# Janspiry/Image-Super-Resolution-via-Iterative-Refinement

Hardware: NVIDIA H100
Metric: diffusion steps/sec (batch16, 16->128 SR3) (higher is better)
Workload: dtype bf16

## Files before the change

image-super-resolution-via-iterative-refinement_b200/_native.py:

```python
import ctypes
import os
from ctypes import POINTER, c_char_p, c_double, c_float, c_int, c_int64, c_uint64, c_void_p

import torch

_PKG = os.path.dirname(os.path.abspath(__file__))
LIB_PATH = os.path.join(_PKG, "lib", "libsr3_b200.so")
SR3_MAX_LEVELS = 8
_lib = None


class NativeLibraryError(RuntimeError):
    pass


class UNetConfigC(ctypes.Structure):
    _fields_ = [("in_channel", c_int), ("out_channel", c_int), ("inner_channel", c_int), ("norm_groups", c_int),
                ("n_mults", c_int), ("channel_mults", c_int * SR3_MAX_LEVELS), ("n_attn_res", c_int),
                ("attn_res", c_int * SR3_MAX_LEVELS), ("res_blocks", c_int), ("image_size", c_int), ("channels", c_int),
                ("conditional", c_int), ("precision", c_int)]


PRECISIONS = {"bf16": 0, "fp32": 1}

# ... 66 lines not shown
    "sr3_windowed_begin": (c_int, [c_void_p, c_void_p, c_void_p, c_uint64, c_uint64, c_void_p]),
    "sr3_windowed_set_snapshots": (c_int, [c_void_p, c_void_p, c_int]),
    "sr3_windowed_steps": (c_int, [c_void_p, c_int, c_int, c_void_p, c_void_p]),
    "sr3_windowed_read_state": (c_int, [c_void_p, c_void_p, c_void_p]),
    "sr3_windowed_grid": (c_int, [c_void_p, POINTER(c_int), POINTER(c_int), POINTER(c_int), POINTER(c_int), POINTER(c_float), POINTER(c_float)]),
    "sr3_windowed_profile_step": (c_int, [c_void_p, c_int, c_int, POINTER(c_float), c_void_p]),
    "sr3_windowed_create_range": (c_int, [c_void_p, c_int, c_int, c_int, c_int, c_int, c_int, c_int, c_void_p, POINTER(c_int), POINTER(c_void_p)]),
    "sr3_windowed_phase_begin": (c_int, [c_void_p, c_int, c_void_p]),
    "sr3_windowed_phase_means": (c_int, [c_void_p, c_void_p]),
    "sr3_windowed_phase_merge": (c_int, [c_void_p, c_void_p]),
    "sr3_wstream_create": (c_int, [c_void_p, c_uint64, c_int, c_int, POINTER(c_void_p)]),
    "sr3_wstream_destroy": (None, [c_void_p]),
    "sr3_wstream_admit": (c_int, [c_void_p, POINTER(c_int), c_int, c_void_p, c_void_p, c_int, c_int, c_uint64, POINTER(c_int), c_void_p]),
    "sr3_wstream_step": (c_int, [c_void_p, c_void_p]),
    "sr3_wstream_retire": (c_int, [c_void_p, c_int, c_void_p]),
    "sr3_wstream_slot_state": (c_int, [c_void_p, POINTER(c_int), POINTER(c_int), POINTER(c_int)]),
    "sr3_engine_profile_step": (c_int, [c_void_p, c_int, c_int, c_int, POINTER(c_int), POINTER(c_float), POINTER(c_double), POINTER(c_double),
                                        POINTER(c_int), c_void_p]),
    "sr3_pil_bicubic_tables": (c_int, [c_int, c_int, POINTER(c_int), POINTER(c_int), c_int, POINTER(c_int)]),
    "sr3_resize_bicubic_u8": (c_int, [c_void_p, c_void_p, c_void_p, c_int, c_int, c_int, c_int, c_int, c_int, c_int, c_float, c_float, c_void_p]),
    "sr3_tensor2img": (c_int, [c_void_p, c_void_p, c_int, c_int, c_int, c_int, c_int, c_float, c_float, c_void_p]),
    "sr3_ssd_u8": (c_int, [c_void_p, c_void_p, c_int64, POINTER(c_uint64), c_void_p]),
    "sr3_ssim": (c_int, [c_void_p, c_void_p, c_int, c_int, c_int, c_int, c_int, POINTER(c_double), c_void_p]),
    "sr3_image_metrics": (c_int, [c_void_p, c_void_p, c_int, c_int, c_int, c_int, c_float, c_float, c_void_p, c_void_p, POINTER(c_uint64),
                                  POINTER(c_double), c_void_p]),
    "sr3_engine_num_launches_per_step": (c_int, [c_void_p]),
    "sr3_engine_num_ops_per_step": (c_int, [c_void_p]),
    "sr3_engine_workspace_bytes": (c_int64, [c_void_p]),
    "sr3_engine_read_activation": (c_int, [c_void_p, c_char_p, c_void_p, c_int64, POINTER(c_int64), POINTER(c_int), c_void_p]),
    "sr3_test_read_gradient": (c_int, [c_void_p, c_char_p, c_int, c_void_p, c_int64, POINTER(c_int64), POINTER(c_int), c_void_p]),
    "sr3_bench_conv": (c_int, [c_int, c_int, c_int, c_int, c_int, c_int, c_int, c_int, c_int, c_int, POINTER(c_float)]),
    "sr3_test_gemm": (c_int, [c_void_p, c_void_p, c_void_p, c_int, c_int, c_int, c_int, c_void_p]),
    "sr3_test_attention": (c_int, [c_void_p, c_void_p, c_void_p, c_int, c_int, c_int, c_int, c_void_p]),
    "sr3_test_conv_groupnorm": (c_int, [c_void_p, c_void_p, c_void_p, c_void_p, c_void_p, c_int, c_int, c_void_p, c_void_p, c_int, c_int, c_int, c_int, c_int,
                                        c_int, c_void_p]),
    "sr3_test_conv": (c_int, [c_void_p, c_void_p, c_void_p, c_void_p, c_void_p, c_int, c_int, c_int, c_int, c_int, c_int, c_int,
                              c_void_p]),
    "sr3_test_conv_ex": (c_int, [POINTER(TestConvArgsC), POINTER(GemmGeometryC), c_void_p]),
    "sr3_tile_schedule": (c_int, [c_void_p, c_int, POINTER(GemmGeometryC), POINTER(c_int), POINTER(c_int)]),
    "sr3_test_wgrad": (c_int, [c_void_p, c_void_p, c_void_p, c_int, c_int, c_int, c_int, c_int, c_int, c_int, c_int, c_int, c_int, c_float,
                               c_int, POINTER(c_int), c_void_p]),
    "sr3_test_groupnorm_layer": (c_int, [POINTER(TestGroupNormArgsC), c_void_p]),
    "sr3_test_grad_combine": (c_int, [c_void_p, c_void_p, c_void_p, c_int, c_void_p, c_void_p, c_void_p, c_void_p, c_float, c_int, c_int, c_int,
                                      c_void_p]),
    "sr3_test_dgrad": (c_int, [c_void_p, c_void_p, c_void_p, c_int, c_int, c_int, c_int, c_int, c_int, c_int, c_int, c_void_p]),
    "sr3_test_attention_bwd": (c_int, [c_void_p, c_void_p, c_void_p, c_void_p, c_void_p, c_void_p, c_void_p, c_void_p, c_int, c_int, c_int, c_int,
                                       c_void_p]),
    "sr3_test_film_embed_bwd": (c_int, [POINTER(TestFilmArgsC), c_void_p]),
    "sr3_test_film_embed_fwd": (c_int, [c_void_p] * 10 + [c_int, c_int, c_int, c_void_p]),
    "sr3_test_attention_unfused": (c_int, [c_void_p] * 5 + [c_int] * 5 + [c_void_p]),
    "sr3_test_loss_grad": (c_int, [c_void_p, c_void_p, c_int, c_int, c_int, c_int, c_int, POINTER(c_double), c_void_p, c_int, c_void_p, c_void_p]),
    "sr3_test_grad_load": (c_int, [c_void_p, c_int, c_int, c_int, c_int, c_void_p, c_int, c_void_p, c_void_p]),
    "sr3_test_noise_level_bwd": (c_int, [c_void_p] * 6 + [c_int, c_int, c_void_p]),
    "sr3_test_input_grad": (c_int, [c_void_p, c_void_p, c_void_p, c_int, c_int, c_int, c_int, c_int, c_void_p]),
}
EXPORTED_SYMBOLS = tuple(_SIGS.keys())


def lib():
    global _lib
    if _lib is not None:
        return _lib
    if not os.path.exists(LIB_PATH):
        raise NativeLibraryError(
            f"{LIB_PATH} is missing: run `python -c 'import __graft_entry__ as g; g.build()'` (nvcc, sm_90a). "
            "sr3_b200 has no CPU or eager-PyTorch fallback.")
# ... 603 lines not shown

    def step(self, n=1):
        with torch.cuda.device(self.device):
            for _ in range(int(n)):
                _check(lib().sr3_wstream_step(self._h, _stream()))

    def slot_state(self):
        r, t, st = (c_int * self.slots)(), (c_int * self.slots)(), (c_int * self.slots)()
        _check(lib().sr3_wstream_slot_state(self._h, r, t, st))
        return list(r), list(t), list(st)

    def finished(self):
        r, _, st = self.slot_state()
        return sorted({q for q, v in zip(r, st) if v == 2})

    def retire(self, request):
        with torch.cuda.device(self.device):
            _check(lib().sr3_wstream_retire(self._h, int(request), _stream()))
        return self._canvases.pop(int(request))[0]


def bench_conv(B, H, W, Cin, Cout, k=3, stride=1, resid=False, stats=True, reps=20):
    ms = c_float()
    _check(lib().sr3_bench_conv(B, H, W, Cin, Cout, k, stride, int(resid), int(stats), reps, ctypes.byref(ms)))
    return ms.value


def test_attention(qk_bf16, vT_bf16, nz, Lt, HW, C):
    out = torch.empty(nz * Lt, C, device=qk_bf16.device, dtype=torch.bfloat16)
    _check(lib().sr3_test_attention(_ptr(qk_bf16), _ptr(vT_bf16), _ptr(out), nz, Lt, HW, C, _stream()))
    return out


def test_gemm(a_bf16, b_bf16, block_n):
    M, K = a_bf16.shape
    N = b_bf16.shape[0]
    d = torch.empty(M, N, device=a_bf16.device, dtype=torch.float32)
    _check(lib().sr3_test_gemm(_ptr(a_bf16), _ptr(b_bf16), _ptr(d), M, N, K, block_n, _stream()))
    return d


def test_conv(x_nhwc_bf16, w_oihw, bias, ksize, stride, want_stats=False):
    B, H, W, Cin = x_nhwc_bf16.shape
    Cout = w_oihw.shape[0]
    y = torch.empty(B, H // stride, W // stride, Cout, device=x_nhwc_bf16.device, dtype=torch.float32)
    stats = torch.zeros(B, Cout, 2, device=y.device, dtype=torch.float64) if want_stats else None
    _check(lib().sr3_test_conv(_ptr(x_nhwc_bf16), _ptr(w_oihw), _ptr(bias), _ptr(y), _ptr(stats), B, H, W, Cin, Cout, ksize, stride, _stream()))
    return y, stats


def test_conv_ex(x, w, ksize=3, stride=1, bias=None, bias2=None, resid=None, x2=None, w2=None, want_bf16=False, want_stats=False,
                 fold_up=False, precise=False):
    B, H, W, CX = x.shape
    Cin = CX // 2 if precise else CX
    Cout = w.shape[0]
    OH, OW = (2 * H, 2 * W) if fold_up else (H // stride, W // stride)
    y = torch.empty(B, OH, OW, Cout, device=x.device, dtype=torch.float32)
    yb = torch.empty(B, OH, OW, Cout * (2 if precise else 1), device=x.device, dtype=torch.bfloat16) if want_bf16 else None
    stats = torch.zeros(B, Cout, 2, device=x.device, dtype=torch.float64) if want_stats else None
    keep = [_f32c(t, x.device) if t is not None else None for t in (w, bias, bias2, resid, w2)]
    a = TestConvArgsC()
    a.x, a.w, a.bias, a.bias2, a.resid = x.data_ptr(), *[(t.data_ptr() if t is not None else None) for t in keep[:4]]
    a.x2 = x2.data_ptr() if x2 is not None else None
    a.w2 = keep[4].data_ptr() if keep[4] is not None else None
    a.y, a.y_bf16, a.stats = y.data_ptr(), (yb.data_ptr() if yb is not None else None), (stats.data_ptr() if stats is not None else None)
    a.B, a.H, a.W, a.Cin, a.Cout = B, H, W, Cin, Cout
# ... 183 lines not shown
```

image-super-resolution-via-iterative-refinement_b200/csrc/attn_long_wgmma.cuh:

```cuda
#pragma once
#include "attn_wgmma.cuh"

namespace sr3 {

constexpr int ATTNL_KB = 128;
constexpr int ATTNL_DN = 128;
constexpr int ATTNL_STAGES = 5;
constexpr int ATTNL_STAGE_BYTES = 16384 + 16384;
constexpr int ATTNL_P_BYTES = 128 * ATTNL_KB * 2;
constexpr int ATTNL_SMEM_BYTES = 1024 + GEMM_HDR_BYTES + ATTNL_STAGES * ATTNL_STAGE_BYTES + ATTNL_P_BYTES;

__global__ void __launch_bounds__(ATTN_THREADS, 1) attn_long_kernel(const __grid_constant__ AttnParams p) {
    extern __shared__ uint8_t smem_raw[];
    const uint32_t raw = smem_u32(smem_raw);
    const uint32_t bar_base = (raw + 1023u) & ~1023u;
    const uint32_t base = bar_base + GEMM_HDR_BYTES;
    const uint32_t p_base = base + ATTNL_STAGES * ATTNL_STAGE_BYTES;
    uint8_t* p_ptr = smem_raw + (p_base - raw);
    auto full_bar = [&](int s) { return bar_base + 8u * s; };
    auto empty_bar = [&](int s) { return bar_base + 8u * (ATTNL_STAGES + s); };

    const int n_dc = p.C / ATTNL_DN;
    const int qt = blockIdx.x / n_dc, dc = blockIdx.x % n_dc, z = blockIdx.y;
    const int warp = threadIdx.x >> 5;
    const int lane = threadIdx.x & 31;
    const int kc1 = p.C / 64;
    constexpr int kc3 = ATTNL_KB / 64;
    const int nb = p.Lt / ATTNL_KB;

    if (threadIdx.x == 0) {
        tma_prefetch_desc(&p.qk_map);
        tma_prefetch_desc(&p.vt_map);
        for (int s = 0; s < ATTNL_STAGES; ++s) { mbar_init(full_bar(s), 1); mbar_init(empty_bar(s), 2); }
        fence_mbar_init();
    }
    __syncthreads();
    pdl_launch_dependents();
    pdl_wait();

    if (warp == ATTN_PRODUCER_WARP) {
        int s = 0;
        uint32_t ph = 0;
        auto stage = [&](bool is_s, int kb, int c) {
            mbar_wait(empty_bar(s), ph ^ 1u);
            if (elect_one_sync()) {
// ... 120 lines not shown
```

image-super-resolution-via-iterative-refinement_b200/csrc/attn_wgmma.cuh:

```cuda
#pragma once
#include <cuda_bf16.h>
#include <cuda.h>
#include "gemm_wgmma.cuh"

namespace sr3 {

constexpr int ATTN_THREADS = 288;
constexpr int ATTN_PRODUCER_WARP = 8;
constexpr int ATTN_STAGES = 3;
constexpr int ATTN_STAGE_BYTES = 16384 + 32768;
constexpr int ATTN_P_BYTES = 65536;
constexpr int ATTN_SMEM_BYTES = 1024 + GEMM_HDR_BYTES + ATTN_STAGES * ATTN_STAGE_BYTES + ATTN_P_BYTES;

struct AttnParams {
    CUtensorMap qk_map;
    CUtensorMap vt_map;
    __nv_bfloat16* out;
    int C, Lt, HW, dn, nz;
    float scale_log2e;
};

template <int LT, int DN>
__device__ __forceinline__ void attn_unit_t(const AttnParams& p, const AttnParams* pm, const uint32_t base_in, uint8_t* base_ptr_in,
                                            const int qt, const int dc, const int z) {
    const uint32_t bar_base = base_in;
    const uint32_t base = base_in + GEMM_HDR_BYTES;
    uint8_t* base_ptr = base_ptr_in + GEMM_HDR_BYTES;
    const uint32_t p_base = base + ATTN_STAGES * ATTN_STAGE_BYTES;
    uint8_t* p_ptr = base_ptr + ATTN_STAGES * ATTN_STAGE_BYTES;
    auto full_bar = [&](int s) { return bar_base + 8u * s; };
    auto empty_bar = [&](int s) { return bar_base + 8u * (ATTN_STAGES + s); };

    const int warp = threadIdx.x >> 5;
    const int lane = threadIdx.x & 31;
    const int kc1 = p.C / 64;
    constexpr int kc3 = LT / 64;

    if (threadIdx.x == 0) {
        tma_prefetch_desc(&pm->qk_map);
        tma_prefetch_desc(&pm->vt_map);
        for (int s = 0; s < ATTN_STAGES; ++s) { mbar_init(full_bar(s), 1); mbar_init(empty_bar(s), 2); }
        fence_mbar_init();
    }
    __syncthreads();
    pdl_launch_dependents();
    pdl_wait();

    if (warp == ATTN_PRODUCER_WARP) {
        int s = 0;
        uint32_t ph = 0;
        for (int it = 0; it < kc1 + kc3; ++it) {
            mbar_wait(empty_bar(s), ph ^ 1u);
            if (elect_one_sync()) {
                const uint32_t dst = base + s * ATTN_STAGE_BYTES;
                if (it < kc1) {
                    mbar_arrive_expect_tx(full_bar(s), 16384 + LT * 128);
                    tma_load_2d(dst, &pm->qk_map, full_bar(s), it * 64, z * LT + qt * 128);
                    for (int j = 0; j < LT / 128; ++j)
                        tma_load_2d(dst + 16384 + j * 16384, &pm->qk_map, full_bar(s), p.C + it * 64, z * LT + j * 128);
                } else {
                    mbar_arrive_expect_tx(full_bar(s), DN * 128);
                    for (int j = 0; j < DN / 128; ++j)
                        tma_load_2d(dst + 16384 + j * 16384, &pm->vt_map, full_bar(s), (it - kc1) * 64, z * p.C + dc * DN + j * 128);
                }
            }
            __syncwarp();
            if (++s == ATTN_STAGES) { s = 0; ph ^= 1u; }
        }
    } else if (warp < ATTN_PRODUCER_WARP) {
        const int g = warp >> 2;
        const int wq = warp & 3;
        const bool leader = (threadIdx.x & 127) == 0;
        int s = 0, prev = -1;
        uint32_t ph = 0;
        auto release_prev = [&]() {
            if (prev >= 0) {
                wgmma_wait<1>();
                mbar_arrive_if(empty_bar(prev), leader);
            }
            prev = s;
            if (++s == ATTN_STAGES) { s = 0; ph ^= 1u; }
        };
        float sacc[LT / 2];
        for (int it = 0; it < kc1; ++it) {
            mbar_wait(full_bar(s), ph);
            wgmma_fence();
            const uint32_t st = base + s * ATTN_STAGE_BYTES;
#pragma unroll
            for (int kk = 0; kk < 4; ++kk)
                Wgmma<LT>::template mma<0, 0>(sacc, wgmma_desc_sw128(st + g * 8192 + kk * 32, 16, 1024), wgmma_desc_sw128(st + 16384 + kk * 32, 16, 1024),
                                              (it | kk) != 0);
            wgmma_commit();
            release_prev();
        }
        wgmma_wait<0>();
        wgmma_fence_regs(sacc);
        int rows[2], segs[2];
        float mx[2] = {-3.0e38f, -3.0e38f}, sum[2] = {0.f, 0.f};
#pragma unroll
        for (int h = 0; h < 2; ++h) {
            rows[h] = 64 * g + 16 * wq + (lane >> 2) + 8 * h;
            segs[h] = (qt * 128 + rows[h]) / p.HW;
        }
#pragma unroll
        for (int j = 0; j < LT / 2; ++j) {
            const int h = (j >> 1) & 1, key = 8 * (j >> 2) + 2 * (lane & 3) + (j & 1);
            if (key / p.HW == segs[h]) mx[h] = fmaxf(mx[h], sacc[j]);
        }
#pragma unroll
        for (int h = 0; h < 2; ++h) {
            mx[h] = fmaxf(mx[h], __shfl_xor_sync(0xffffffffu, mx[h], 1));
            mx[h] = fmaxf(mx[h], __shfl_xor_sync(0xffffffffu, mx[h], 2));
        }
        const float mxs[2] = {mx[0] * p.scale_log2e, mx[1] * p.scale_log2e};
#pragma unroll
        for (int j = 0; j < LT / 2; j += 2) {
            const int h = (j >> 1) & 1, key = 8 * (j >> 2) + 2 * (lane & 3);
            const float x0 = exp2f(fmaf(sacc[j], p.scale_log2e, -mxs[h])), x1 = exp2f(fmaf(sacc[j + 1], p.scale_log2e, -mxs[h]));
            const float e0 = (key / p.HW == segs[h]) ? x0 : 0.f, e1 = ((key + 1) / p.HW == segs[h]) ? x1 : 0.f;
            sum[h] += e0 + e1;
            const int r = rows[h];
            uint8_t* dst = p_ptr + (key >> 6) * 16384 + (r >> 3) * 1024 + (r & 7) * 128 + ((((key & 63) >> 3) ^ (r & 7)) << 4) + (key & 7) * 2;
            *reinterpret_cast<__nv_bfloat162*>(dst) = __floats2bfloat162_rn(e0, e1);
        }
#pragma unroll
        for (int h = 0; h < 2; ++h) {
            sum[h] += __shfl_xor_sync(0xffffffffu, sum[h], 1);
            sum[h] += __shfl_xor_sync(0xffffffffu, sum[h], 2);
        }
        fence_proxy_async_smem();
        asm volatile("bar.sync %0, 128;" ::"r"(2 + g) : "memory");

        float oacc[DN / 2];
        for (int kc = 0; kc < kc3; ++kc) {
            mbar_wait(full_bar(s), ph);
            wgmma_fence();
            const uint32_t st = base + s * ATTN_STAGE_BYTES;
            const uint32_t pa = p_base + kc * 16384 + g * 8192;
#pragma unroll
            for (int kk = 0; kk < 4; ++kk)
                Wgmma<DN>::template mma<0, 0>(oacc, wgmma_desc_sw128(pa + kk * 32, 16, 1024), wgmma_desc_sw128(st + 16384 + kk * 32, 16, 1024),
                                              (kc | kk) != 0);
            wgmma_commit();
            release_prev();
        }
        wgmma_wait<0>();
        wgmma_fence_regs(oacc);
        if (prev >= 0) mbar_arrive_if(empty_bar(prev), leader);
        const float inv[2] = {1.0f / sum[0], 1.0f / sum[1]};
#pragma unroll
        for (int j = 0; j < DN / 2; j += 2) {
            const int h = (j >> 1) & 1, col = 8 * (j >> 2) + 2 * (lane & 3);
            __nv_bfloat16* o = p.out + (static_cast<long long>(z) * LT + qt * 128 + rows[h]) * p.C + dc * DN + col;
            *reinterpret_cast<__nv_bfloat162*>(o) = __floats2bfloat162_rn(oacc[j] * inv[h], oacc[j + 1] * inv[h]);
        }
    }
    __syncthreads();
}

__device__ __forceinline__ void attn_unit(const AttnParams& p, const AttnParams* pm, const uint32_t base, uint8_t* base_ptr, const int qt,
                                          const int dc, const int z) {
    if (p.Lt == 256) {
        if (p.dn == 256) attn_unit_t<256, 256>(p, pm, base, base_ptr, qt, dc, z);
        else attn_unit_t<256, 128>(p, pm, base, base_ptr, qt, dc, z);
    } else {
        if (p.dn == 256) attn_unit_t<128, 256>(p, pm, base, base_ptr, qt, dc, z);
        else attn_unit_t<128, 128>(p, pm, base, base_ptr, qt, dc, z);
    }
}

__global__ void __launch_bounds__(ATTN_THREADS, 1) attn_kernel(const __grid_constant__ AttnParams p) {
    extern __shared__ uint8_t smem_raw[];
    const uint32_t raw = smem_u32(smem_raw);
    const uint32_t base = (raw + 1023u) & ~1023u;
    const int n_dc = p.C / p.dn;
    attn_unit(p, &p, base, smem_raw + (base - raw), blockIdx.x / n_dc, blockIdx.x % n_dc, blockIdx.y);
}

}
```

image-super-resolution-via-iterative-refinement_b200/csrc/engine.cu:

```cuda
#include <cuda.h>
#include <cuda_runtime.h>

#include <cmath>
#include <cstdarg>
#include <cstdlib>
#include <cstring>
#include <functional>
#include <limits>
#include <map>
#include <memory>
#include <mutex>
#include <stdexcept>
#include <string>
#include <vector>

#include "../../include/sr3_b200.h"
#include "aux_kernels.cuh"
#include "attn_wgmma.cuh"
#include "attn_long_wgmma.cuh"
#include "train_kernels.cuh"
#include "window_kernels.cuh"
#include "window_stream_kernels.cuh"

using namespace sr3;
// ... 389 lines not shown
    REQUIRE((bn == 16 || bn == 32 || bn == 64 || bn == 128 || bn == 256) && (mh == 1 || (mh == 2 && bn <= 128 && bn != 32)), "unsupported tile %dx%d", 128 * mh, bn);
    const bool pp = d.pingpong != 0;
    REQUIRE(!pp || (gemm_pingpong_ok(bn, mh) && p.ksplit == 1 && d.mode == 0), "no ping-pong form of tile %dx%d (split %d)", 128 * mh, bn, p.ksplit);
    if (geo) {
        geo->tall = d.tall; geo->mh = mh; geo->block_n = bn; geo->h_box = d.h_box; geo->b_box = d.b_box;
        geo->ksplit = p.ksplit; geo->stages = p.stages; geo->ctas = ctas; geo->tiles = total_tiles / p.ksplit; geo->res_smem = res_smem ? 1 : 0;
    }
    if (schedule) *schedule = pp ? 1 : 0;
    std::shared_ptr<GemmParams> sp = std::make_shared<GemmParams>(p);
    if (g_gemm_registry) {
        GemmHandle h; h.p = sp; h.w_ptr = d.b_ptr; h.w_bytes = 2LL * d.b_rows * d.b_K; h.w_is_param = d.b_is_param; h.bn = bn; h.mh = mh;
        g_gemm_registry->push_back(h);
    }
    return [sp, grid, bn, mh, pp, smem](cudaStream_t st) {
        const GemmParams& p = *sp;
        if (pp) {
            if (mh == 2) launch_gemm_bn<64, 2, true>(p, grid, smem, st);
            else if (bn == 64) launch_gemm_bn<64, 1, true>(p, grid, smem, st);
            else launch_gemm_bn<128, 1, true>(p, grid, smem, st);
            return;
        }
        switch (bn) {
            case 16: if (mh == 2) launch_gemm_bn<16, 2>(p, grid, smem, st); else launch_gemm_bn<16, 1>(p, grid, smem, st); break;
            case 32: launch_gemm_bn<32, 1>(p, grid, smem, st); break;
            case 64: if (mh == 2) launch_gemm_bn<64, 2>(p, grid, smem, st); else launch_gemm_bn<64, 1>(p, grid, smem, st); break;
            case 128: if (mh == 2) launch_gemm_bn<128, 2>(p, grid, smem, st); else launch_gemm_bn<128, 1>(p, grid, smem, st); break;
            default: launch_gemm_bn<256, 1>(p, grid, smem, st); break;
        }
    };
}

bool attn_fusable(int Lt, int C) { return Lt >= 128 && Lt % 128 == 0 && C % 128 == 0 && C >= 128; }

Op make_attn_op(const bf16* qk, const bf16* vT, bf16* out, int nz, int Lt, int HW, int C) {
    REQUIRE(attn_fusable(Lt, C) && Lt % HW == 0, "attention shape Lt=%d HW=%d C=%d is not supported by the fused kernel", Lt, HW, C);
    REQUIRE(Lt <= 256 || HW == Lt, "attention over %d tokens per batch takes one image per batch (HW=%d)", Lt, HW);
    AttnParams p;
    memset(&p, 0, sizeof(p));
    {
        const uint64_t dims[2] = {(uint64_t)2 * C, (uint64_t)nz * Lt};
        const uint64_t str[1] = {(uint64_t)2 * C * 2};
        const uint32_t box[2] = {64u, 128u};
        p.qk_map = encode_map(2, qk, dims, str, box);
    }
    {
        const uint64_t dims[2] = {(uint64_t)Lt, (uint64_t)nz * C};
        const uint64_t str[1] = {(uint64_t)Lt * 2};
        const uint32_t box[2] = {64u, 128u};
        p.vt_map = encode_map(2, vT, dims, str, box);
    }
    p.out = out; p.C = C; p.Lt = Lt; p.HW = HW; p.nz = nz;
    p.dn = (C % 256 == 0) ? 256 : 128;
    p.scale_log2e = 1.4426950408889634f / sqrtf((float)C);
    if (Lt > 256) {
        p.dn = ATTNL_DN;
        static std::vector<int> seen_long;
        if (first_use_on_device(seen_long)) CK(cudaFuncSetAttribute(attn_long_kernel, cudaFuncAttributeMaxDynamicSharedMemorySize, ATTNL_SMEM_BYTES));
        const dim3 grid((Lt / 128) * (C / ATTNL_DN), nz, 1);
        return [p, grid](cudaStream_t st) { launch_k(attn_long_kernel, grid, dim3(ATTN_THREADS), ATTNL_SMEM_BYTES, st, p); };
    }
    static std::vector<int> seen;
    if (first_use_on_device(seen)) CK(cudaFuncSetAttribute(attn_kernel, cudaFuncAttributeMaxDynamicSharedMemorySize, ATTN_SMEM_BYTES));
    const dim3 grid((Lt / 128) * (C / p.dn), nz, 1);
    return [p, grid](cudaStream_t st) { launch_k(attn_kernel, grid, dim3(ATTN_THREADS), ATTN_SMEM_BYTES, st, p); };
}

void pick_image_box(int W, int H, int& w_box, int& h_box, int& b_box);
int pick_block_n(int cout);
int pingpong_knob() {
    const char* e = getenv("SR3_PINGPONG");
    return e ? (atoi(e) != 0 ? 1 : 0) : -1;
}

void conv_geometry(GemmDesc& d, int OW, int OH, int Bt, int cout, bool has_resid = false, int nz = 1) {
    const int npass = d.passes > 1 ? d.passes : 1;
    bool tall_ok = OW >= 8 && OH >= 16, has3 = false;
    for (const KSlab& k : d.slabs) { if (k.p != 0) tall_ok = false; if (k.dh != 0) has3 = true; }
    tall_ok = tall_ok && has3 && (OH >= 32 || Bt % 2 == 0);
    const int sms = num_sms();
    const int pp_knob = pingpong_knob();
    const bool pp_force = pp_knob == 1, pp_auto = pp_knob < 0;
    const bool shape_forced = getenv("SR3_TALL_BN") || getenv("SR3_TALL_MH") || getenv("SR3_BLOCK_N");
    constexpr double EPI_COOP = 200000.0, EPI_COOP_256x128 = 2000000.0, EPI_PP_128REG = 600000.0;
    const double EPI_PP_64REG = tall_ok ? 200000.0 : 10000.0;
    auto items_of = [](int rows, int bn) { return (double)(rows / 128) * (bn >= 32 ? bn / 32 : 1); };
    auto model = [&](long long tiles, int nstage, long long stage_bytes, int rows, int bn, int& split, bool pp = false) -> double {
        if (pp) {
            split = 1;
            const long long t = (tiles + sms - 1) / sms;
            const double mma = (double)nstage * stage_bytes, epi = items_of(rows, bn) * (rows == 128 && bn == 64 ? EPI_PP_64REG : EPI_PP_128REG);
            const double serial = (double)t * mma + epi, paired = (double)((t + 1) / 2) * (mma + epi);
            return serial > paired ? serial : paired;
        }
        int smax = 1;
        if (bn >= 32 && cout % 32 == 0) {
            smax = (int)(sms / tiles);
            const int units = (rows / 128) * (bn / 32) * 4;
// ... 2113 lines not shown
            CK(cudaMemcpyAsync(hb.data(), a.gb, n * sizeof(uint16_t), cudaMemcpyDeviceToHost, st));
            CK(cudaStreamSynchronize(st));
            for (int64_t i = 0; i < n; ++i) hf[i] = (uint32_t)hb[i] << 16;
            CK(cudaMemcpyAsync(dst, hf.data(), n * 4, cudaMemcpyHostToDevice, st));
        }
        CK(cudaStreamSynchronize(st));
    }
    API_END
}

int sr3_test_gemm(const void* a, const void* b, float* dptr, int M, int N, int K, int block_n, void* stream) {
    API_BEGIN
    REQUIRE(M % 128 == 0 && K % 64 == 0 && N % block_n == 0, "bad test gemm shape");
    DevAllocs mem;
    GemmDesc d; d.n_a = 1; d.a[0] = matrix_src(a, 1, M, K, K, 0);
    for (int c = 0; c < K; c += 64) d.slabs.push_back({0, c, 0, 0, 0, c});
    d.block_n = block_n; d.b_ptr = b; d.b_K = K; d.b_rows = N;
    d.w_box = 128; d.h_box = 1; d.b_box = 1; d.tiles_w = M / 128; d.tiles_h = 1; d.tiles_b = 1; d.n_tiles = N / block_n; d.nz = 1;
    d.OW = M; d.OH = 1; d.OB = 1; d.n_valid = N;
    d.out_f32 = dptr; d.os = OutSpec{0, 0, 0, N, 0};
    Op op = make_gemm_op(d, mem);
    cudaStream_t st = static_cast<cudaStream_t>(stream);
    op(st);
    CK(cudaStreamSynchronize(st));
    API_END
}

int sr3_test_attention(const void* qk, const void* vT, void* out, int nz, int Lt, int HW, int C, void* stream) {
    API_BEGIN
    Op op = make_attn_op(static_cast<const bf16*>(qk), static_cast<const bf16*>(vT), static_cast<bf16*>(out), nz, Lt, HW, C);
    cudaStream_t st = static_cast<cudaStream_t>(stream);
    op(st);
    CK(cudaStreamSynchronize(st));
    API_END
}

int sr3_test_attention_unfused(const void* qk, const void* vT, float* S, void* P, void* O, int nz, int Lt, int HW, int C, int precise,
                               void* stream) {
    API_BEGIN
    REQUIRE(qk && vT && S && P && O, "null argument");
    REQUIRE(nz >= 1 && Lt % 128 == 0 && C % 128 == 0 && HW >= 1 && Lt % HW == 0, "unfused attention geometry Lt=%d HW=%d C=%d", Lt, HW, C);
    const int PW = precise ? 2 : 1;
    cudaStream_t st = static_cast<cudaStream_t>(stream);
    DevAllocs mem;
    make_gemm_op(attn_s_desc(static_cast<const bf16*>(qk), S, nz, Lt, C, PW), mem)(st);
    launch_softmax(attn_softmax_params(S, static_cast<bf16*>(P), nz, Lt, HW, PW), st);
    make_gemm_op(attn_pv_desc(static_cast<const bf16*>(P), static_cast<const bf16*>(vT), static_cast<bf16*>(O), nz, Lt, C, PW), mem)(st);
    CK(cudaStreamSynchronize(st));
    API_END
}

int sr3_bench_conv(int B, int H, int W, int Cin, int Cout, int ksize, int stride, int with_resid, int with_stats, int reps, float* ms_out) {
    API_BEGIN
    REQUIRE(ms_out && reps > 0, "bad arguments");
    DevAllocs mem;
    const int ktot = ksize * ksize * Cin;
    const int OH = H / stride, OW = W / stride;
    bf16* x = static_cast<bf16*>(mem.alloc((size_t)B * H * W * Cin * 2));
    bf16* wp = static_cast<bf16*>(mem.alloc((size_t)Cout * ktot * 2));
    float* y = static_cast<float*>(mem.alloc((size_t)B * OH * OW * Cout * 4));
    float* r = with_resid ? static_cast<float*>(mem.alloc((size_t)B * OH * OW * Cout * 4)) : nullptr;
    double* st = with_stats ? static_cast<double*>(mem.alloc((size_t)B * Cout * 2 * 8)) : nullptr;
    float* bias = static_cast<float*>(mem.alloc((size_t)Cout * 4));
    GemmDesc d; d.n_a = 1;
    d.a[0] = stride == 1 ? nhwc_src(x, B, H, W, Cin) : nhwc_stride2_src(x, B, H, W, Cin);
    add_conv_slabs(d.slabs, 0, Cin, ksize, stride, 0);
// ... 551 lines not shown
```

include/sr3_b200.h:

```cpp
#ifndef SR3_B200_H
#define SR3_B200_H

#include <stdint.h>

#ifdef __cplusplus
extern "C" {
#endif

#define SR3_MAX_LEVELS 8

typedef struct sr3_unet_config {
    int in_channel;
    int out_channel;
    int inner_channel;
    int norm_groups;
    int n_mults;
    int channel_mults[SR3_MAX_LEVELS];
    int n_attn_res;
    int attn_res[SR3_MAX_LEVELS];
    int res_blocks;
    int image_size;
    int channels;
    int conditional;
    int precision;
// ... 73 lines not shown
int sr3_windowed_phase_begin(sr3_windowed* w, int t_start, void* stream);
int sr3_windowed_phase_means(sr3_windowed* w, void* stream);
int sr3_windowed_phase_merge(sr3_windowed* w, void* stream);

typedef struct sr3_wstream sr3_wstream;
int sr3_wstream_create(sr3_engine* e, uint64_t seed, int overlap_h, int overlap_w, sr3_wstream** out);
void sr3_wstream_destroy(sr3_wstream* s);
int sr3_wstream_admit(sr3_wstream* s, const int* slots, int n_slots, const float* condition_x, float* x, int height, int width,
                      uint64_t sample_index, int* request, void* stream);
int sr3_wstream_step(sr3_wstream* s, void* stream);
int sr3_wstream_retire(sr3_wstream* s, int request, void* stream);
int sr3_wstream_slot_state(const sr3_wstream* s, int* request, int* t, int* state);

int sr3_tensor2img(const float* src, unsigned char* dst_u8, int n, int C, int H, int W, int nrow, float min_v, float max_v, void* stream);
int sr3_ssd_u8(const unsigned char* a_u8, const unsigned char* b_u8, int64_t n, unsigned long long* ssd_host, void* stream);
int sr3_ssim(const void* a, const void* b, int dtype, int n, int H, int W, int C, double* ssim_host, void* stream);
int sr3_image_metrics(const float* sr_f32, const float* hr_f32, int n, int C, int H, int W, float min_v, float max_v, unsigned char* sr_u8,
                      unsigned char* hr_u8, unsigned long long* ssd_host, double* ssim_host, void* stream);

int sr3_pil_bicubic_tables(int in_size, int out_size, int* bounds, int* coef, int coef_cap, int* ksize);
int sr3_resize_bicubic_u8(const unsigned char* src_u8, unsigned char* dst_u8, float* dst_f32, int B, int h, int w, int C, int H, int W, int flip,
                          float min_v, float max_v, void* stream);

int sr3_engine_num_launches_per_step(const sr3_engine* e);
int sr3_engine_num_ops_per_step(const sr3_engine* e);
int64_t sr3_engine_workspace_bytes(const sr3_engine* e);
int sr3_engine_profile_step(sr3_engine* e, int t, int reps, int cap, int* kinds, float* ms, double* flops, double* bytes, int* n_ops,
                            void* stream);
int sr3_engine_read_activation(sr3_engine* e, const char* name, float* dst, int64_t cap, int64_t* numel, int shape_bhwc[4], void* stream);
int sr3_test_read_gradient(sr3_engine* e, const char* name, int form, float* dst, int64_t cap, int64_t* numel, int shape_bhwc[4], void* stream);

int sr3_test_gemm(const void* a_bf16, const void* b_bf16, float* d, int M, int N, int K, int block_n, void* stream);
int sr3_test_attention(const void* qk_bf16, const void* vT_bf16, void* out_bf16, int nz, int Lt, int HW, int C, void* stream);
int sr3_test_attention_unfused(const void* qk_bf16, const void* vT_bf16, float* S, void* P_bf16, void* O_bf16, int nz, int Lt, int HW, int C,
                               int precise, void* stream);
int sr3_test_conv(const void* x_bf16, const float* w_oihw, const float* bias, float* y, double* stats, int B, int H, int W, int Cin,
                  int Cout, int ksize, int stride, void* stream);

typedef struct sr3_gemm_geometry {
    int tall, mh, block_n, h_box, b_box, ksplit, stages, ctas, tiles, res_smem;
} sr3_gemm_geometry;
typedef struct sr3_test_conv_args {
    const void* x; const float* w; const float* bias; const float* bias2; const float* resid;
    const void* x2; const float* w2;
    float* y; void* y_bf16; double* stats;
    int B, H, W, Cin, Cout, Cin2, ksize, stride;
    int fold_up, precise;
} sr3_test_conv_args;
int sr3_test_conv_ex(const sr3_test_conv_args* args, sr3_gemm_geometry* geometry, void* stream);
int sr3_tile_schedule(const sr3_engine* e, int op, sr3_gemm_geometry* geometry, int* schedule, int* out_hwc);
int sr3_test_wgrad(const void* dy_bf16, const void* x_bf16, float* grad, int B, int OH, int OW, int CY, int Cin, int ksize, int stride,
                   int cout_valid, int cin_valid, int slices, float gscale, int raw, int* slices_used, void* stream);

int sr3_test_conv_groupnorm(const void* x_bf16, const float* w_oihw, const float* bias, const float* gamma, const float* beta, int groups,
                            int silu, float* y, void* a_bf16, int B, int H, int W, int Cin, int Cout, int ksize, void* stream);


typedef struct sr3_test_groupnorm_args {
    const float* x0; const float* x1; const double* st0; const double* st1; const float* gamma; const float* beta;
    const unsigned char* drop_mask; const float* dA; const float* add;
    void* a_bf16; float* mr; float* dst0; void* dst0_b; float* gsum0; float* dst1; float* dgamma; float* dbeta;
    uint64_t drop_seed;
    int B, HW, C0, C1, groups, silu, drop, add_ld, acc0;
    unsigned int drop_layer;
    float drop_p, gscale;
} sr3_test_groupnorm_args;
int sr3_test_groupnorm_layer(const sr3_test_groupnorm_args* args, void* stream);
int sr3_test_grad_combine(const float* a, const float* b, float* dst, int acc, void* dst_b, float* gsum, float* bias0, float* bias1, float gscale,
                          int B, int HW, int C, void* stream);
int sr3_test_dgrad(const void* dy_bf16, const float* w_oihw, float* dx, int form, int B, int H, int W, int CY, int Cin, int Cout, int ksize,
                   void* stream);
int sr3_test_attention_bwd(const void* qk_bf16, const void* vT_bf16, const void* P_bf16, const void* dO_bf16, float* dS, void* dS_bf16, float* dqkv,
                           void* dqkv_bf16, int nz, int Lt, int HW, int C, void* stream);
typedef struct sr3_test_film_args {
    const float* wf; const float* tau; const float* dfilm; const float* nl; const float* w1; const float* b1; const float* w2;
    float* dwf; float* dbf; float* dcb; float* dtau; float* dw1; float* db1; float* dw2; float* db2;
    int F, inner, B;
    float gscale;
} sr3_test_film_args;
int sr3_test_film_embed_bwd(const sr3_test_film_args* args, void* stream);
int sr3_test_film_embed_fwd(const float* nl, const float* w1, const float* b1, const float* w2, const float* b2, const float* wf, const float* bf,
                            const float* cb, float* tau, float* film, int F, int inner, int B, void* stream);
int sr3_test_loss_grad(const float* noise, const float* eps, int B, int C, int H, int W, int l2, double* loss_host, void* deps_bf16, int ld,
                       float* bias_sum, void* stream);
int sr3_test_grad_load(const float* g, int B, int C, int H, int W, void* deps_bf16, int ld, float* bias_sum, void* stream);
int sr3_test_noise_level_bwd(const float* nl, const float* w1, const float* b1, const float* w2, const float* dtau, float* dnl, int inner, int B,
                             void* stream);
int sr3_test_input_grad(const void* dy_bf16, const float* w_oihw, float* dx, int B, int H, int W, int inner, int in_channel, void* stream);

int sr3_bench_conv(int B, int H, int W, int Cin, int Cout, int ksize, int stride, int with_resid, int with_stats, int reps, float* ms_out);

#ifdef __cplusplus
}
#endif
#endif
```

Measured before the change: 149.5.

## Template attention kernel, add warp-specialized register rebalancing and wave-aware channel slicing

The fused short-sequence attention kernel becomes a template kernel over sequence length and channel slice, so runtime dispatch is removed. It grows to three warpgroups and uses setmaxnreg to give the consumer warps more registers while shrinking the producer warps. A new heuristic picks the channel slice (64, 128 or 256) that keeps the fewest CTA waves across the SMs, so small grids fill the GPU better. The cross-image mask now sets scores to -inf before the max, which drops the per-element integer divisions. Test and benchmark entry points are also added, at the cost of more template instantiations and idle extra warps.

```diff
diff --git a/image-super-resolution-via-iterative-refinement_b200/_native.py b/image-super-resolution-via-iterative-refinement_b200/_native.py
--- a/image-super-resolution-via-iterative-refinement_b200/_native.py
+++ b/image-super-resolution-via-iterative-refinement_b200/_native.py
@@ -122,6 +122,9 @@
     "sr3_bench_conv": (c_int, [c_int, c_int, c_int, c_int, c_int, c_int, c_int, c_int, c_int, c_int, POINTER(c_float)]),
     "sr3_test_gemm": (c_int, [c_void_p, c_void_p, c_void_p, c_int, c_int, c_int, c_int, c_void_p]),
     "sr3_test_attention": (c_int, [c_void_p, c_void_p, c_void_p, c_int, c_int, c_int, c_int, c_void_p]),
+    "sr3_test_attention_dn": (c_int, [c_void_p, c_void_p, c_void_p, c_int, c_int, c_int, c_int, c_int, c_void_p]),
+    "sr3_attention_dn": (c_int, [c_int, c_int, c_int, c_int, POINTER(c_int)]),
+    "sr3_bench_attention": (c_int, [c_void_p, c_void_p, c_void_p, c_int, c_int, c_int, c_int, c_int, c_int, POINTER(c_float)]),
     "sr3_test_conv_groupnorm": (c_int, [c_void_p, c_void_p, c_void_p, c_void_p, c_void_p, c_int, c_int, c_void_p, c_void_p, c_int, c_int, c_int, c_int, c_int,
                                         c_int, c_void_p]),
     "sr3_test_conv": (c_int, [c_void_p, c_void_p, c_void_p, c_void_p, c_void_p, c_int, c_int, c_int, c_int, c_int, c_int, c_int,
@@ -791,6 +794,26 @@
     return out
 
 
+def test_attention_dn(qk_bf16, vT_bf16, nz, Lt, HW, C, dn):
+    out = torch.empty(nz * Lt, C, device=qk_bf16.device, dtype=torch.bfloat16)
+    _check(lib().sr3_test_attention_dn(_ptr(qk_bf16), _ptr(vT_bf16), _ptr(out), nz, Lt, HW, C, dn, _stream()))
+    return out
+
+
+def attention_dn(nz, Lt, C, sms=0):
+    dn = c_int()
+    _check(lib().sr3_attention_dn(nz, Lt, C, sms, ctypes.byref(dn)))
+    return dn.value
+
+
+def bench_attention(qk_bf16, vT_bf16, nz, Lt, HW, C, dn=0, reps=50):
+    out = torch.empty(nz * Lt, C, device=qk_bf16.device, dtype=torch.bfloat16)
+    ms = c_float()
+    torch.cuda.synchronize()
+    _check(lib().sr3_bench_attention(_ptr(qk_bf16), _ptr(vT_bf16), _ptr(out), nz, Lt, HW, C, dn, reps, ctypes.byref(ms)))
+    return ms.value, out
+
+
 def test_gemm(a_bf16, b_bf16, block_n):
     M, K = a_bf16.shape
     N = b_bf16.shape[0]
diff --git a/image-super-resolution-via-iterative-refinement_b200/csrc/attn_long_wgmma.cuh b/image-super-resolution-via-iterative-refinement_b200/csrc/attn_long_wgmma.cuh
--- a/image-super-resolution-via-iterative-refinement_b200/csrc/attn_long_wgmma.cuh
+++ b/image-super-resolution-via-iterative-refinement_b200/csrc/attn_long_wgmma.cuh
@@ -3,6 +3,7 @@
 
 namespace sr3 {
 
+constexpr int ATTNL_THREADS = 288;
 constexpr int ATTNL_KB = 128;
 constexpr int ATTNL_DN = 128;
 constexpr int ATTNL_STAGES = 5;
@@ -10,7 +11,7 @@
 constexpr int ATTNL_P_BYTES = 128 * ATTNL_KB * 2;
 constexpr int ATTNL_SMEM_BYTES = 1024 + GEMM_HDR_BYTES + ATTNL_STAGES * ATTNL_STAGE_BYTES + ATTNL_P_BYTES;
 
-__global__ void __launch_bounds__(ATTN_THREADS, 1) attn_long_kernel(const __grid_constant__ AttnParams p) {
+__global__ void __launch_bounds__(ATTNL_THREADS, 1) attn_long_kernel(const __grid_constant__ AttnParams p) {
     extern __shared__ uint8_t smem_raw[];
     const uint32_t raw = smem_u32(smem_raw);
     const uint32_t bar_base = (raw + 1023u) & ~1023u;
diff --git a/image-super-resolution-via-iterative-refinement_b200/csrc/attn_wgmma.cuh b/image-super-resolution-via-iterative-refinement_b200/csrc/attn_wgmma.cuh
--- a/image-super-resolution-via-iterative-refinement_b200/csrc/attn_wgmma.cuh
+++ b/image-super-resolution-via-iterative-refinement_b200/csrc/attn_wgmma.cuh
@@ -5,8 +5,13 @@
 
 namespace sr3 {
 
-constexpr int ATTN_THREADS = 288;
+constexpr int ATTN_THREADS = 384;
+constexpr int ATTN_CONSUMER_WARPS = 8;
 constexpr int ATTN_PRODUCER_WARP = 8;
+constexpr int ATTN_CONSUMER_REGS = 232;
+constexpr int ATTN_PRODUCER_REGS = 40;
+static_assert(ATTN_CONSUMER_WARPS * 32 * ATTN_CONSUMER_REGS + (ATTN_THREADS - ATTN_CONSUMER_WARPS * 32) * ATTN_PRODUCER_REGS <= 65536, "register file");
+static_assert(ATTN_THREADS == 384 && ATTN_PRODUCER_WARP == ATTN_CONSUMER_WARPS, "setmaxnreg acts on whole warpgroups: 2 consumer + 1 producer");
 constexpr int ATTN_STAGES = 3;
 constexpr int ATTN_STAGE_BYTES = 16384 + 32768;
 constexpr int ATTN_P_BYTES = 65536;
@@ -21,11 +26,16 @@
 };
 
 template <int LT, int DN>
-__device__ __forceinline__ void attn_unit_t(const AttnParams& p, const AttnParams* pm, const uint32_t base_in, uint8_t* base_ptr_in,
-                                            const int qt, const int dc, const int z) {
-    const uint32_t bar_base = base_in;
-    const uint32_t base = base_in + GEMM_HDR_BYTES;
-    uint8_t* base_ptr = base_ptr_in + GEMM_HDR_BYTES;
+__global__ void __launch_bounds__(ATTN_THREADS, 1) attn_kernel(const __grid_constant__ AttnParams p) {
+    static_assert((LT == 128 || LT == 256) && (DN == 64 || DN == 128 || DN == 256), "attn_kernel shape");
+    constexpr int VB = DN < 128 ? DN : 128;
+    extern __shared__ uint8_t smem_raw[];
+    const uint32_t raw = smem_u32(smem_raw);
+    const uint32_t bar_base = (raw + 1023u) & ~1023u;
+    const uint32_t base = bar_base + GEMM_HDR_BYTES;
+    uint8_t* base_ptr = smem_raw + (base - raw);
+    const int n_dc = p.C / DN;
+    const int qt = blockIdx.x / n_dc, dc = blockIdx.x % n_dc, z = blockIdx.y;
     const uint32_t p_base = base + ATTN_STAGES * ATTN_STAGE_BYTES;
     uint8_t* p_ptr = base_ptr + ATTN_STAGES * ATTN_STAGE_BYTES;
     auto full_bar = [&](int s) { return bar_base + 8u * s; };
@@ -37,8 +47,8 @@
     constexpr int kc3 = LT / 64;
 
     if (threadIdx.x == 0) {
-        tma_prefetch_desc(&pm->qk_map);
-        tma_prefetch_desc(&pm->vt_map);
+        tma_prefetch_desc(&p.qk_map);
+        tma_prefetch_desc(&p.vt_map);
         for (int s = 0; s < ATTN_STAGES; ++s) { mbar_init(full_bar(s), 1); mbar_init(empty_bar(s), 2); }
         fence_mbar_init();
     }
@@ -46,7 +56,9 @@
     pdl_launch_dependents();
     pdl_wait();
 
-    if (warp == ATTN_PRODUCER_WARP) {
+    if (warp >= ATTN_CONSUMER_WARPS) {
+        setmaxnreg_dec<ATTN_PRODUCER_REGS>();
+        if (warp != ATTN_PRODUCER_WARP) return;
         int s = 0;
         uint32_t ph = 0;
         for (int it = 0; it < kc1 + kc3; ++it) {
@@ -55,19 +67,20 @@
                 const uint32_t dst = base + s * ATTN_STAGE_BYTES;
                 if (it < kc1) {
                     mbar_arrive_expect_tx(full_bar(s), 16384 + LT * 128);
-                    tma_load_2d(dst, &pm->qk_map, full_bar(s), it * 64, z * LT + qt * 128);
+                    tma_load_2d(dst, &p.qk_map, full_bar(s), it * 64, z * LT + qt * 128);
                     for (int j = 0; j < LT / 128; ++j)
-                        tma_load_2d(dst + 16384 + j * 16384, &pm->qk_map, full_bar(s), p.C + it * 64, z * LT + j * 128);
+                        tma_load_2d(dst + 16384 + j * 16384, &p.qk_map, full_bar(s), p.C + it * 64, z * LT + j * 128);
                 } else {
                     mbar_arrive_expect_tx(full_bar(s), DN * 128);
-                    for (int j = 0; j < DN / 128; ++j)
-                        tma_load_2d(dst + 16384 + j * 16384, &pm->vt_map, full_bar(s), (it - kc1) * 64, z * p.C + dc * DN + j * 128);
+                    for (int j = 0; j < DN / VB; ++j)
+                        tma_load_2d(dst + 16384 + j * VB * 128, &p.vt_map, full_bar(s), (it - kc1) * 64, z * p.C + dc * DN + j * VB);
                 }
             }
             __syncwarp();
             if (++s == ATTN_STAGES) { s = 0; ph ^= 1u; }
         }
-    } else if (warp < ATTN_PRODUCER_WARP) {
+    } else {
+        setmaxnreg_inc<ATTN_CONSUMER_REGS>();
         const int g = warp >> 2;
         const int wq = warp & 3;
         const bool leader = (threadIdx.x & 127) == 0;
@@ -95,17 +108,19 @@
         }
         wgmma_wait<0>();
         wgmma_fence_regs(sacc);
-        int rows[2], segs[2];
+        int rows[2], seg0[2];
         float mx[2] = {-3.0e38f, -3.0e38f}, sum[2] = {0.f, 0.f};
 #pragma unroll
         for (int h = 0; h < 2; ++h) {
             rows[h] = 64 * g + 16 * wq + (lane >> 2) + 8 * h;
-            segs[h] = (qt * 128 + rows[h]) / p.HW;
+            seg0[h] = (qt * 128 + rows[h]) / p.HW * p.HW - 2 * (lane & 3);
         }
+        auto same_image = [&](int jkey, int h) { return static_cast<unsigned>(jkey - seg0[h]) < static_cast<unsigned>(p.HW); };
 #pragma unroll
         for (int j = 0; j < LT / 2; ++j) {
-            const int h = (j >> 1) & 1, key = 8 * (j >> 2) + 2 * (lane & 3) + (j & 1);
-            if (key / p.HW == segs[h]) mx[h] = fmaxf(mx[h], sacc[j]);
+            const int h = (j >> 1) & 1;
+            if (!same_image(8 * (j >> 2) + (j & 1), h)) sacc[j] = -INFINITY;
+            mx[h] = fmaxf(mx[h], sacc[j]);
         }
 #pragma unroll
         for (int h = 0; h < 2; ++h) {
@@ -116,8 +131,7 @@
 #pragma unroll
         for (int j = 0; j < LT / 2; j += 2) {
             const int h = (j >> 1) & 1, key = 8 * (j >> 2) + 2 * (lane & 3);
-            const float x0 = exp2f(fmaf(sacc[j], p.scale_log2e, -mxs[h])), x1 = exp2f(fmaf(sacc[j + 1], p.scale_log2e, -mxs[h]));
-            const float e0 = (key / p.HW == segs[h]) ? x0 : 0.f, e1 = ((key + 1) / p.HW == segs[h]) ? x1 : 0.f;
+            const float e0 = exp2f(fmaf(sacc[j], p.scale_log2e, -mxs[h])), e1 = exp2f(fmaf(sacc[j + 1], p.scale_log2e, -mxs[h]));
             sum[h] += e0 + e1;
             const int r = rows[h];
             uint8_t* dst = p_ptr + (key >> 6) * 16384 + (r >> 3) * 1024 + (r & 7) * 128 + ((((key & 63) >> 3) ^ (r & 7)) << 4) + (key & 7) * 2;
@@ -155,26 +169,6 @@
             *reinterpret_cast<__nv_bfloat162*>(o) = __floats2bfloat162_rn(oacc[j] * inv[h], oacc[j + 1] * inv[h]);
         }
     }
-    __syncthreads();
-}
-
-__device__ __forceinline__ void attn_unit(const AttnParams& p, const AttnParams* pm, const uint32_t base, uint8_t* base_ptr, const int qt,
-                                          const int dc, const int z) {
-    if (p.Lt == 256) {
-        if (p.dn == 256) attn_unit_t<256, 256>(p, pm, base, base_ptr, qt, dc, z);
-        else attn_unit_t<256, 128>(p, pm, base, base_ptr, qt, dc, z);
-    } else {
-        if (p.dn == 256) attn_unit_t<128, 256>(p, pm, base, base_ptr, qt, dc, z);
-        else attn_unit_t<128, 128>(p, pm, base, base_ptr, qt, dc, z);
-    }
-}
-
-__global__ void __launch_bounds__(ATTN_THREADS, 1) attn_kernel(const __grid_constant__ AttnParams p) {
-    extern __shared__ uint8_t smem_raw[];
-    const uint32_t raw = smem_u32(smem_raw);
-    const uint32_t base = (raw + 1023u) & ~1023u;
-    const int n_dc = p.C / p.dn;
-    attn_unit(p, &p, base, smem_raw + (base - raw), blockIdx.x / n_dc, blockIdx.x % n_dc, blockIdx.y);
 }
 
 }
diff --git a/image-super-resolution-via-iterative-refinement_b200/csrc/engine.cu b/image-super-resolution-via-iterative-refinement_b200/csrc/engine.cu
--- a/image-super-resolution-via-iterative-refinement_b200/csrc/engine.cu
+++ b/image-super-resolution-via-iterative-refinement_b200/csrc/engine.cu
@@ -445,11 +445,35 @@
 
 bool attn_fusable(int Lt, int C) { return Lt >= 128 && Lt % 128 == 0 && C % 128 == 0 && C >= 128; }
 
-Op make_attn_op(const bf16* qk, const bf16* vT, bf16* out, int nz, int Lt, int HW, int C) {
+int attn_pick_dn(int nz, int Lt, int C, int sms) {
+    int best = 0;
+    long long best_waves = 0;
+    for (int dn : {256, 128, 64}) {
+        if (C % dn != 0) continue;
+        const long long ctas = (long long)(Lt / 128) * (C / dn) * nz;
+        const long long waves = (ctas + sms - 1) / sms;
+        if (best == 0 || waves <= best_waves) { best = dn; best_waves = waves; }
+    }
+    return best;
+}
+
+template <int LT, int DN>
+Op attn_op_t(const AttnParams& p, dim3 grid) {
+    static std::vector<int> seen;
+    if (first_use_on_device(seen)) CK(cudaFuncSetAttribute(attn_kernel<LT, DN>, cudaFuncAttributeMaxDynamicSharedMemorySize, ATTN_SMEM_BYTES));
+    return [p, grid](cudaStream_t st) { launch_k(attn_kernel<LT, DN>, grid, dim3(ATTN_THREADS), ATTN_SMEM_BYTES, st, p); };
+}
+
+Op make_attn_op(const bf16* qk, const bf16* vT, bf16* out, int nz, int Lt, int HW, int C, int dn = 0) {
     REQUIRE(attn_fusable(Lt, C) && Lt % HW == 0, "attention shape Lt=%d HW=%d C=%d is not supported by the fused kernel", Lt, HW, C);
     REQUIRE(Lt <= 256 || HW == Lt, "attention over %d tokens per batch takes one image per batch (HW=%d)", Lt, HW);
+    REQUIRE(dn == 0 || (Lt <= 256 && (dn == 64 || dn == 128 || dn == 256) && C % dn == 0),
+            "attention channel slice dn=%d is not supported for Lt=%d C=%d", dn, Lt, C);
     AttnParams p;
     memset(&p, 0, sizeof(p));
+    p.out = out; p.C = C; p.Lt = Lt; p.HW = HW; p.nz = nz;
+    p.dn = Lt > 256 ? ATTNL_DN : dn ? dn : attn_pick_dn(nz, Lt, C, num_sms());
+    p.scale_log2e = 1.4426950408889634f / sqrtf((float)C);
     {
         const uint64_t dims[2] = {(uint64_t)2 * C, (uint64_t)nz * Lt};
         const uint64_t str[1] = {(uint64_t)2 * C * 2};
@@ -459,23 +483,23 @@
     {
         const uint64_t dims[2] = {(uint64_t)Lt, (uint64_t)nz * C};
         const uint64_t str[1] = {(uint64_t)Lt * 2};
-        const uint32_t box[2] = {64u, 128u};
+        const uint32_t box[2] = {64u, (uint32_t)(p.dn < 128 ? p.dn : 128)};
         p.vt_map = encode_map(2, vT, dims, str, box);
     }
-    p.out = out; p.C = C; p.Lt = Lt; p.HW = HW; p.nz = nz;
-    p.dn = (C % 256 == 0) ? 256 : 128;
-    p.scale_log2e = 1.4426950408889634f / sqrtf((float)C);
+    const dim3 grid((Lt / 128) * (C / p.dn), nz, 1);
     if (Lt > 256) {
-        p.dn = ATTNL_DN;
         static std::vector<int> seen_long;
         if (first_use_on_device(seen_long)) CK(cudaFuncSetAttribute(attn_long_kernel, cudaFuncAttributeMaxDynamicSharedMemorySize, ATTNL_SMEM_BYTES));
-        const dim3 grid((Lt / 128) * (C / ATTNL_DN), nz, 1);
-        return [p, grid](cudaStream_t st) { launch_k(attn_long_kernel, grid, dim3(ATTN_THREADS), ATTNL_SMEM_BYTES, st, p); };
-    }
-    static std::vector<int> seen;
-    if (first_use_on_device(seen)) CK(cudaFuncSetAttribute(attn_kernel, cudaFuncAttributeMaxDynamicSharedMemorySize, ATTN_SMEM_BYTES));
-    const dim3 grid((Lt / 128) * (C / p.dn), nz, 1);
-    return [p, grid](cudaStream_t st) { launch_k(attn_kernel, grid, dim3(ATTN_THREADS), ATTN_SMEM_BYTES, st, p); };
+        return [p, grid](cudaStream_t st) { launch_k(attn_long_kernel, grid, dim3(ATTNL_THREADS), ATTNL_SMEM_BYTES, st, p); };
+    }
+    if (Lt == 256) {
+        if (p.dn == 256) return attn_op_t<256, 256>(p, grid);
+        if (p.dn == 128) return attn_op_t<256, 128>(p, grid);
+        return attn_op_t<256, 64>(p, grid);
+    }
+    if (p.dn == 256) return attn_op_t<128, 256>(p, grid);
+    if (p.dn == 128) return attn_op_t<128, 128>(p, grid);
+    return attn_op_t<128, 64>(p, grid);
 }
 
 void pick_image_box(int W, int H, int& w_box, int& h_box, int& b_box);
@@ -2655,6 +2679,50 @@
     cudaStream_t st = static_cast<cudaStream_t>(stream);
     op(st);
     CK(cudaStreamSynchronize(st));
+    API_END
+}
+
+int sr3_test_attention_dn(const void* qk, const void* vT, void* out, int nz, int Lt, int HW, int C, int dn, void* stream) {
+    API_BEGIN
+    Op op = make_attn_op(static_cast<const bf16*>(qk), static_cast<const bf16*>(vT), static_cast<bf16*>(out), nz, Lt, HW, C, dn);
+    cudaStream_t st = static_cast<cudaStream_t>(stream);
+    op(st);
+    CK(cudaStreamSynchronize(st));
+    API_END
+}
+
+int sr3_attention_dn(int nz, int Lt, int C, int sms, int* dn_out) {
+    API_BEGIN
+    REQUIRE(dn_out && nz > 0 && attn_fusable(Lt, C), "bad arguments");
+    *dn_out = Lt > 256 ? ATTNL_DN : attn_pick_dn(nz, Lt, C, sms > 0 ? sms : num_sms());
+    API_END
+}
+
+int sr3_bench_attention(const void* qk, const void* vT, void* out, int nz, int Lt, int HW, int C, int dn, int reps, float* ms_out) {
+    API_BEGIN
+    REQUIRE(ms_out && reps > 0, "bad arguments");
+    Op op = make_attn_op(static_cast<const bf16*>(qk), static_cast<const bf16*>(vT), static_cast<bf16*>(out), nz, Lt, HW, C, dn);
+    cudaStream_t cs;
+    CK(cudaStreamCreateWithFlags(&cs, cudaStreamNonBlocking));
+    for (int i = 0; i < 3; ++i) op(cs);
+    CK(cudaStreamSynchronize(cs));
+    cudaGraph_t g; cudaGraphExec_t ge;
+    CK(cudaStreamBeginCapture(cs, cudaStreamCaptureModeThreadLocal));
+    for (int i = 0; i < reps; ++i) op(cs);
+    CK(cudaStreamEndCapture(cs, &g));
+    CK(cudaGraphInstantiate(&ge, g, 0));
+    CK(cudaGraphLaunch(ge, cs));
+    CK(cudaStreamSynchronize(cs));
+    cudaEvent_t e0, e1;
+    CK(cudaEventCreate(&e0)); CK(cudaEventCreate(&e1));
+    CK(cudaEventRecord(e0, cs));
+    CK(cudaGraphLaunch(ge, cs));
+    CK(cudaEventRecord(e1, cs));
+    CK(cudaEventSynchronize(e1));
+    float ms = 0; CK(cudaEventElapsedTime(&ms, e0, e1));
+    cudaGraphExecDestroy(ge); cudaGraphDestroy(g); cudaStreamDestroy(cs);
+    cudaEventDestroy(e0); cudaEventDestroy(e1);
+    *ms_out = ms / reps;
     API_END
 }
 
diff --git a/include/sr3_b200.h b/include/sr3_b200.h
--- a/include/sr3_b200.h
+++ b/include/sr3_b200.h
@@ -129,6 +129,8 @@
 
 int sr3_test_gemm(const void* a_bf16, const void* b_bf16, float* d, int M, int N, int K, int block_n, void* stream);
 int sr3_test_attention(const void* qk_bf16, const void* vT_bf16, void* out_bf16, int nz, int Lt, int HW, int C, void* stream);
+int sr3_test_attention_dn(const void* qk_bf16, const void* vT_bf16, void* out_bf16, int nz, int Lt, int HW, int C, int dn, void* stream);
+int sr3_attention_dn(int nz, int Lt, int C, int sms, int* dn);
 int sr3_test_attention_unfused(const void* qk_bf16, const void* vT_bf16, float* S, void* P_bf16, void* O_bf16, int nz, int Lt, int HW, int C,
                                int precise, void* stream);
 int sr3_test_conv(const void* x_bf16, const float* w_oihw, const float* bias, float* y, double* stats, int B, int H, int W, int Cin,
@@ -186,6 +188,7 @@
 int sr3_test_input_grad(const void* dy_bf16, const float* w_oihw, float* dx, int B, int H, int W, int inner, int in_channel, void* stream);
 
 int sr3_bench_conv(int B, int H, int W, int Cin, int Cout, int ksize, int stride, int with_resid, int with_stats, int reps, float* ms_out);
+int sr3_bench_attention(const void* qk_bf16, const void* vT_bf16, void* out_bf16, int nz, int Lt, int HW, int C, int dn, int reps, float* ms_out);
 
 #ifdef __cplusplus
 }
```

After: 154.1 (median of 6 runs). 1.03x the previous value.
